# Lumina-Group/libzkp

Measured on AMD Instinct MI355X. Metric: proofs/sec (whole node) + ms/proof p50, 4096-proof mixed batch (range / equality / membership / improvement) per MI355X, higher is better.
Workload: dtype u32/u64 integer limbs (10x25.5-bit GF(2^255-19), BN254 Fq on 9x29-bit limbs in the MSM loops and 10x26-bit elsewhere, 8x32-bit Fr and scalars mod l, 2x64-bit f128)

## Files before the change

libzkp_amd/csrc/batch_impl.inc:

```
namespace {

struct PackView {
    uint32_t n;
    const uint64_t* src_off;
    const uint32_t* len_fixed;
    const uint32_t* dyn_ix;
    const uint8_t* dyn_kind;
    const int32_t* status_fixed;
    const uint32_t* dyn_len; const int32_t* dyn_status;
    uint32_t* len; int32_t* status; uint64_t* out_off;
    const uint8_t* arena; uint8_t* out;
};
__global__ void __launch_bounds__(256) k_batch_lens(PackView P) {
    const uint32_t i = blockIdx.x * 256 + threadIdx.x;
    if (i >= P.n) return;
    int32_t st = P.status_fixed[i];
    uint32_t l = P.len_fixed[i];
    if (st == 0 && l == LEN_DYN) {
        const uint32_t k = P.dyn_ix[i];
        l = P.dyn_len[k];
        if (P.dyn_kind[i] == DYN_LEN_STATUS) st = P.dyn_status[k];
        else if (l == 0) st = ZKP_HIP_PROOF_GENERATION_FAILED;
    }
    if (st != 0) l = 0;
// ... 190 lines not shown
    hipStream_t st = dev().stream;
    if (P.in_bytes) HIP_TRY(hipMemcpyAsync(P.d_in, h, P.in_bytes, hipMemcpyHostToDevice, st));
    HIP_TRY(hipStreamSynchronize(st));
    return 0;
}

PackView pack_view(const ShardPlan& P) {
    uint8_t *in = P.d_in, *ar = P.d_arena;
    PackView V{};
    V.n = P.n; V.src_off = (const uint64_t*)(in + P.i_src); V.len_fixed = (const uint32_t*)(in + P.i_lenf); V.dyn_ix = (const uint32_t*)(in + P.i_dix);
    V.dyn_kind = in + P.i_dkind; V.status_fixed = (const int32_t*)(in + P.i_stf); V.dyn_len = (const uint32_t*)(ar + P.a_dlen); V.dyn_status = (const int32_t*)(ar + P.a_dst);
    V.len = (uint32_t*)(P.d_meta + P.m_len); V.status = (int32_t*)(P.d_meta + P.m_status); V.out_off = (uint64_t*)(P.d_meta + P.m_off);
    V.arena = ar; V.out = P.d_out;
    return V;
}

int launch_shard_enqueue(ShardPlan& P) {
    BatchState* BS = nullptr; int rc;
    if ((rc = batch_state(&BS))) return rc;
    const uint32_t n = P.n;
    uint32_t lane_ix = 0;
    if ((rc = pick_lane(*BS, &lane_ix))) return rc;
    BatchLane& LN = BS->lane[lane_ix];
    hipStream_t st = LN.main;
    uint8_t *in = P.d_in, *ar = P.d_arena;
    const VariantPlan &R = P.var[ZKP_HIP_OP_RANGE], &E = P.var[ZKP_HIP_OP_EQUALITY], &T = P.var[ZKP_HIP_OP_THRESHOLD], &M = P.var[ZKP_HIP_OP_MEMBERSHIP],
                      &I = P.var[ZKP_HIP_OP_IMPROVEMENT], &C = P.var[ZKP_HIP_OP_CONSISTENCY];
    trace_origin(st);
    if (P.arena_bytes) HIP_TRY(hipMemsetAsync(ar, 0, P.arena_bytes, st));
    if (T.rows) HIP_TRY(hipMemcpyAsync(ar + T.arena, P.thr_img.data(), P.thr_img.size(), hipMemcpyHostToDevice, st));
    if (C.rows) HIP_TRY(hipMemcpyAsync(ar + C.arena, P.con_img.data(), P.con_img.size(), hipMemcpyHostToDevice, st));
    HIP_TRY(hipEventRecord(LN.go, st));
    bool used[4] = {false, false, false, false};
    auto on_stream = [&](int k, auto body) -> int {
        hipStream_t s = nullptr; used[k] = true;
        int rcs;
        if ((rcs = lane_stream(*BS, k, &s))) return rcs;
        HIP_TRY(hipStreamWaitEvent(s, LN.go, 0));
        if ((rcs = body(s))) return rcs;
        HIP_TRY(hipEventRecord(LN.done[k], s));
        return 0;
    };
    if (R.rows || T.rows || C.rows) {
        static const int edg_prio = env_int("ZKP_HIP_EDG_PRIORITY", 1);
        struct PrioScope { int& r; PrioScope(int& ref, int v) : r(ref) { r = v; } ~PrioScope() { r = 0; } };
        PrioScope prio(dev().msm_prio_now, (E.rows + M.rows) && edg_prio ? 1 : 0);
        SubBatch& jobs_sb = dev().sub[0];
        if ((rc = on_stream(0, [&](hipStream_t s) -> int {
                int rcb;
                if (R.rows && (rcb = prove_range_device_locked(R.rows, (const uint64_t*)(in + P.i_rv), (const uint64_t*)(in + P.i_rmin), (const uint64_t*)(in + P.i_rmax), 6, in + P.i_rseed,
                                                               ar + R.arena, R.stride, (uint32_t*)(ar + P.a_dlen), (int32_t*)(ar + P.a_dst), s, nullptr, (int)lane_ix))) return rcb;
                if (T.rows && (rcb = run_jobs_on(jobs_sb, P.thrJ, in + P.i_tseed, ar + T.arena, 6, s))) return rcb;
                if (C.rows) {
                    if ((rcb = run_jobs_on(jobs_sb, P.conJ, in + P.i_cseed, ar + C.arena, 6, s))) return rcb;
                    k_consistency_digest<<<(C.rows + 63) / 64, 64, 0, s>>>(ar + C.arena, C.stride, (const uint32_t*)(in + P.i_ccount), (const uint32_t*)(in + P.i_clen), C.rows);
                }
                return 0;
            }))) return rc;
    }
    if (I.rows && (rc = on_stream(3, [&](hipStream_t s) -> int {
            if (const int rcb = ensure_stark_constants()) return rcb;
            ZKP_TRACED("k_stark_prove", s, stark_launch_prove((const uint64_t*)(in + P.i_io), (const uint64_t*)(in + P.i_in), I.rows, g_stark_const, ar + I.arena, I.stride,
                                                              (uint32_t*)(ar + P.a_dlen) + R.rows, s));
            return 0;
        }))) return rc;
    if (M.rows && (rc = on_stream(2, [&](hipStream_t s) {
            return run_g16(G16_MEMBERSHIP, M.rows, (const uint64_t*)(in + P.i_mv), (const uint64_t*)(in + P.i_msets), (const uint32_t*)(in + P.i_mlen), in + P.i_mseed,
                           ar + M.arena, M.stride, s, lane_ix);
        }))) return rc;
    if (E.rows && (rc = on_stream(1, [&](hipStream_t s) {
            return run_g16(G16_EQUALITY, E.rows, (const uint64_t*)(in + P.i_ev), nullptr, nullptr, in + P.i_eseed, ar + E.arena, E.stride, s, lane_ix);
        }))) return rc;
    for (int k = 0; k < 4; k++) if (used[k]) HIP_TRY(hipStreamWaitEvent(st, LN.done[k], 0));
    const PackView V = pack_view(P);
    if (n && P.self_check) {
    } else if (n) {
        ZKP_TRACED("k_batch_lens+scan+pack", st, k_batch_lens<<<(n + 255) / 256, 256, 0, st>>>(V); k_batch_scan<<<1, 1024, 0, st>>>(V); k_batch_pack<<<n, 256, 0, st>>>(V));
    } else {
        HIP_TRY(hipMemsetAsync(P.d_meta + P.m_off, 0, 8, st));
    }
    HIP_TRY(hipGetLastError());
    HIP_TRY(hipEventRecord(P.finished, st));
    HIP_TRY(hipEventRecord(LN.idle, st)); LN.used = true;
    P.in_flight = true;
    return 0;
}
int launch_shard(ShardPlan& P) {
    if (P.generation != dev().generation) return fail(ZKP_HIP_E_ARGUMENT, "the batch was staged before zkp_hip_shutdown: stage it again");
    if (P.var[ZKP_HIP_OP_EQUALITY].rows && !g16s().key[G16_EQUALITY].loaded) return no_proving_key(g16s().key[G16_EQUALITY]);
    if (P.var[ZKP_HIP_OP_MEMBERSHIP].rows && !g16s().key[G16_MEMBERSHIP].loaded) return no_proving_key(g16s().key[G16_MEMBERSHIP]);
    const int rc = launch_shard_enqueue(P);
    if (rc) {
        const std::string keep = t_err;
        (void)hipDeviceSynchronize();
        t_err = keep;
    }
    return rc;
}
int self_check_shard(ShardPlan& P) {
    const auto t0 = std::chrono::steady_clock::now();
    const uint32_t n = P.n;
    hipStream_t st = dev().stream;
    uint8_t *in = P.d_in, *ar = P.d_arena;
    const PackView W = pack_view(P);
    SelfCheckView V{};
// ... 282 lines not shown
```

libzkp_amd/csrc/g16_impl.inc:

```

namespace {

struct G16Key {
    bool loaded = false;
    uint32_t n_inst = 0, n_wit = 0, nv = 0, n_rows = 0, m = 0, logm = 0;
    G16Circuit C{};
    std::vector<void*> allocs;
    uint32_t *table_g1 = nullptr, *table_g2 = nullptr;
    G16Radix rx = g16_radix(G16_WBITS_DEFAULT);
    int shared_tables = -1;
    uint64_t table_bytes = 0;
    struct Chunking { DevLayout lay; const uint32_t* corr = nullptr; const uint16_t* scal = nullptr; };
    std::vector<SlotList> targets_g1, targets_g2;
    std::vector<uint16_t> hscal_g1, hscal_g2;
    std::map<uint64_t, Chunking> lays_g1, lays_g2;
    uint64_t win_g1 = 0, win_g2 = 0;
    const uint32_t *init_g1 = nullptr, *init_g2 = nullptr;
    G16Vk vk{}; bool vk_ready = false;
    uint64_t vk_table_bytes = 0;
    bool verifier_only() const { return vk_ready && !loaded; }
    const uint32_t *vm_kconst = nullptr, *vm_lines = nullptr;
};
struct G16Run {
    void* buf = nullptr; size_t cap = 0; hipStream_t side = nullptr, side2 = nullptr; hipEvent_t ev[4] = {nullptr, nullptr, nullptr, nullptr};
// ... 350 lines not shown
    for (uint32_t k = 0; k < nv; k++) s2.push_back(Bt[k]);
    std::vector<uint8_t> b1, b2; int rc;
    if ((rc = gpu_scalar_mults(false, s1, b1)) || (rc = gpu_scalar_mults(true, s2, b2))) return rc;
    auto g1at = [&](size_t i) { return b1.data() + 64 * i; };
    auto g2at = [&](size_t i) { return b2.data() + 128 * i; };
    auto put = [](std::vector<uint8_t>& v, const uint8_t* p, size_t n) { v.insert(v.end(), p, p + n); };
    auto put_len = [](std::vector<uint8_t>& v, uint64_t n) { for (int i = 0; i < 8; i++) v.push_back((uint8_t)(n >> (8 * i))); };
    size_t o_abc = 3, o_a = o_abc + T.n_inst, o_b = o_a + nv, o_h = o_b + nv, o_l = o_h + (m - 1);
    vk.clear();
    put(vk, g1at(0), 64); put(vk, g2at(0), 128); put(vk, g2at(1), 128); put(vk, g2at(2), 128);
    put_len(vk, T.n_inst); put(vk, g1at(o_abc), 64ull * T.n_inst);
    pk = vk;
    put(pk, g1at(1), 64); put(pk, g1at(2), 64);
    put_len(pk, nv); put(pk, g1at(o_a), 64ull * nv);
    put_len(pk, nv); put(pk, g1at(o_b), 64ull * nv);
    put_len(pk, nv); put(pk, g2at(3), 128ull * nv);
    put_len(pk, m - 1); put(pk, g1at(o_h), 64ull * (m - 1));
    put_len(pk, T.n_wit); put(pk, g1at(o_l), 64ull * T.n_wit);
    return load_key_locked(kind, pk.data(), pk.size());
}

int launch_msm_key(bool g2, const G16Radix& rx, const G16Key::Chunking& ch, const uint32_t* table, const uint32_t* acc_init, uint32_t rows, const uint32_t* digits, uint32_t* partial, hipStream_t st) {
    const DevLayout& D = ch.lay;
    const MsmView m = g16_msm_view(rx, D, ch.scal, table, acc_init, rows, digits, partial);
    Device::KProf& K = dev().prof[g2 ? 2 : 1];
    hipEvent_t e1 = nullptr;
    int rc = prof_begin(K, st, &e1);
    if (rc) return rc;
    ZKP_TRACED(g2 ? "k_msm_gather<G2Msm>" : "k_msm_gather<G1Msm>", st, g16_launch_msm(g2, m, st));
    prof_end(K, st, e1, D.adds_per_row * rows);
    return 0;
}


int run_g16(int kind, uint32_t rows, const uint64_t* d_value, const uint64_t* d_set_vals, const uint32_t* d_set_len, const uint8_t* d_seeds,
            uint8_t* d_out, uint64_t stride, hipStream_t st, uint32_t lane = 0) {
    G16Key& K = g16s().key[kind];
    if (!K.loaded) return no_proving_key(K);
    const uint32_t nsc = g16_nscalars(K.nv, K.m);
    const G16Key::Chunking *c1 = nullptr, *c1c = nullptr, *c2 = nullptr;
    int rc;
    if ((rc = get_chunking(K, false, G16_PART_AB, rows, &c1)) || (rc = get_chunking(K, true, G16_PART_ALL, rows, &c2))) return rc;
    if ((rc = get_chunking(K, false, G16_PART_C, rows, &c1c))) return rc;
    size_t off = 0;
    auto sz = [&](size_t bytes) { size_t o = off; off += align_up(bytes); return o; };
    const size_t W = (size_t)32 * rows;
    const size_t o_z = sz(W * K.nv), o_sd = sz((size_t)K.rx.digw * 4 * rows * nsc), o_rs = sz(W * 2), o_p1 = sz((size_t)c1->lay.nchunks * G1_JAC_W * 4 * rows),
                 o_p1c = sz((size_t)c1c->lay.nchunks * G1_JAC_W * 4 * rows), o_p2 = sz((size_t)c2->lay.nchunks * G2_JAC_W * 4 * rows),
                 o_s1 = sz((size_t)3 * G1_JAC_W * 4 * rows), o_s2 = sz((size_t)G2_JAC_W * 4 * rows), o_t1 = sz((size_t)G16_CPARTS * G1_JAC_W * 4 * rows),
                 o_qe = sz((size_t)2 * 9 * K.m * 4 * rows);
    G16Run& RW = g16s().run[kind][lane & 1u];
    if (off > RW.cap) {
        if (RW.buf) { HIP_TRY(hipDeviceSynchronize()); HIP_TRY(hipFree(RW.buf)); RW.buf = nullptr; RW.cap = 0; }
        HIP_TRY(hipMalloc(&RW.buf, off)); RW.cap = off;
    }
    uint8_t* base = (uint8_t*)RW.buf;
    G16View V{}; V.rx = K.rx; V.rows = rows; V.kind = (uint32_t)kind; V.n_inst = K.n_inst; V.n_wit = K.n_wit; V.nv = K.nv; V.m = K.m;
    V.value = d_value; V.set_vals = d_set_vals; V.set_len = d_set_len; V.seeds = reinterpret_cast<const uint32_t*>(d_seeds); V.mimc_c = g16s().mimc_dev;
    V.z = (uint32_t*)(base + o_z); V.sdig = (uint32_t*)(base + o_sd); V.rs = (uint32_t*)(base + o_rs); V.out = d_out; V.stride = stride;
    V.qap_evals = (uint32_t*)(base + o_qe);
    uint32_t *p1 = (uint32_t*)(base + o_p1), *p1c = (uint32_t*)(base + o_p1c), *p2 = (uint32_t*)(base + o_p2), *s1 = (uint32_t*)(base + o_s1), *s2 = (uint32_t*)(base + o_s2), *t1 = (uint32_t*)(base + o_t1);
    if (!RW.last) {
        for (auto& e : RW.ev) HIP_TRY(hipEventCreateWithFlags(&e, hipEventDisableTiming));
        HIP_TRY(hipEventCreateWithFlags(&RW.last, hipEventDisableTiming));
    }
    G16Run& R0 = g16s().run[kind][0];
    if (!R0.side) {
        static const int side_level = env_int("ZKP_HIP_G16_SIDE_PRIORITY", 2), side2_level = env_int("ZKP_HIP_G16_SIDE2_PRIORITY", 0);
        HIP_TRY(hipStreamCreateWithPriority(&R0.side, hipStreamNonBlocking, stream_priority(side_level)));
        HIP_TRY(hipStreamCreateWithPriority(&R0.side2, hipStreamNonBlocking, stream_priority(side2_level)));
    }
    hipStream_t const side = R0.side, side2 = R0.side2;
    hipEvent_t ev_wit = RW.ev[0], ev_ab = RW.ev[1], ev_c = RW.ev[2], ev_cp = RW.ev[3];
    ReduceView R2{}; R2.rows = rows; R2.ntargets = 1; R2.partial = p2; R2.target_chunk_begin = c2->lay.target_chunk_begin; R2.corr = c2->corr;
    if (RW.used) HIP_TRY(hipStreamWaitEvent(st, RW.last, 0));
    ZKP_TRACED("k_g16_witness", st, g16_launch_witness(V, st));
    ZKP_TRACED("k_g16_zdigits", st, g16_launch_zdigits(V, st));
    HIP_TRY(hipEventRecord(ev_wit, st));
    HIP_TRY(hipStreamWaitEvent(side, ev_wit, 0));
    { TraceMark tm_("k_g16_qap", side); HIP_TRY(g16_launch_qap(V, K.C, side)); }
    if ((rc = launch_msm_key(false, K.rx, *c1c, K.table_g1, K.init_g1, rows, V.sdig, p1c, side))) return rc;
    ReduceView Rc{}; Rc.rows = rows; Rc.ntargets = 1; Rc.partial = p1c; Rc.target_chunk_begin = c1c->lay.target_chunk_begin; Rc.corr = c1c->corr;
    ZKP_TRACED("k_sum_t<G1Msm>", side, g16_launch_sum(false, Rc, s1 + (size_t)2 * G1_JAC_W * rows, side));
    HIP_TRY(hipEventRecord(ev_c, side));
    if ((rc = launch_msm_key(false, K.rx, *c1, K.table_g1, K.init_g1, rows, V.sdig, p1, st))) return rc;
    ReduceView Rab{}; Rab.rows = rows; Rab.ntargets = 2; Rab.partial = p1; Rab.target_chunk_begin = c1->lay.target_chunk_begin; Rab.corr = c1->corr;
    if (c1->lay.ntargets == 3) Rab.target_chunk_end = c1->lay.target_chunk_begin + 2;
    HIP_TRY(hipEventRecord(ev_ab, st));
    HIP_TRY(hipStreamWaitEvent(side2, ev_ab, 0));
    ZKP_TRACED("k_sum_t<G1Msm>", side2, g16_launch_sum(false, Rab, s1, side2));
    ZKP_TRACED("k_g16_cparts", side2, g16_launch_cparts(V, s1, t1, side2));
    HIP_TRY(hipEventRecord(ev_cp, side2));
    if ((rc = launch_msm_key(true, K.rx, *c2, K.table_g2, K.init_g2, rows, V.sdig, p2, st))) return rc;
    ZKP_TRACED("k_sum_t<G2Msm>", st, g16_launch_sum(true, R2, s2, st));
    HIP_TRY(hipStreamWaitEvent(st, ev_c, 0));
    HIP_TRY(hipStreamWaitEvent(st, ev_cp, 0));
    ZKP_TRACED("k_g16_final", st, g16_launch_final(V, s1, s2, t1, st));
    HIP_TRY(hipGetLastError());
    HIP_TRY(hipEventRecord(RW.last, st)); RW.used = true;
    return 0;
}

int prove_g16_host(int kind, uint64_t n, const uint64_t* values, const uint64_t* sets_flat, const uint32_t* set_counts, const std::vector<uint8_t>& valid,
                   const uint8_t* seeds, uint8_t* out, uint64_t stride, uint32_t* out_len, int32_t* status) {
    if (g16s().key[kind].verifier_only()) return no_proving_key(g16s().key[kind]);
    std::vector<uint64_t> v, sv; std::vector<uint32_t> sl, idx; std::vector<uint8_t> sd;
    size_t pos = 0; int any = 0;
    memset(out, 0, stride * n);
    for (uint64_t i = 0; i < n; i++) {
        const uint32_t cnt = set_counts ? set_counts[i] : 0;
        if (valid[i]) {
            idx.push_back((uint32_t)i); v.push_back(values[i]);
            sd.insert(sd.end(), seeds + 32 * i, seeds + 32 * i + 32);
            if (kind == G16_MEMBERSHIP) { sl.push_back(cnt); for (uint32_t k = 0; k < G16_MAX_SET; k++) sv.push_back(k < cnt ? sets_flat[pos + k] : 0); }
            const uint32_t plen = kind == G16_EQUALITY ? EQUALITY_ENVELOPE_BYTES : (uint32_t)membership_envelope_bytes(cnt);
            if (plen > stride) return fail(ZKP_HIP_E_ARGUMENT, "stride too small for the proof envelope");
            out_len[i] = plen; status[i] = ZKP_HIP_OK;
        } else { out_len[i] = 0; status[i] = ZKP_HIP_INVALID_INPUT; any = 1; }
        pos += cnt;
    }
    const uint32_t rows = (uint32_t)idx.size();
    if (rows == 0) return any;
    hipStream_t st = dev().stream;
    uint64_t *d_v = nullptr, *d_sv = nullptr; uint32_t* d_sl = nullptr; uint8_t *d_sd = nullptr, *d_out = nullptr;
    DevScope mem;
    HIP_TRY(mem.alloc(&d_v, 8ull * rows)); HIP_TRY(mem.alloc(&d_sd, 32ull * rows)); HIP_TRY(mem.alloc(&d_out, stride * rows));
    HIP_TRY(hipMemcpyAsync(d_v, v.data(), 8ull * rows, hipMemcpyHostToDevice, st));
    HIP_TRY(hipMemcpyAsync(d_sd, sd.data(), 32ull * rows, hipMemcpyHostToDevice, st));
    HIP_TRY(hipMemsetAsync(d_out, 0, stride * rows, st));
    if (kind == G16_MEMBERSHIP) {
        HIP_TRY(mem.alloc(&d_sv, 8ull * sv.size())); HIP_TRY(mem.alloc(&d_sl, 4ull * rows));
        HIP_TRY(hipMemcpyAsync(d_sv, sv.data(), 8ull * sv.size(), hipMemcpyHostToDevice, st));
        HIP_TRY(hipMemcpyAsync(d_sl, sl.data(), 4ull * rows, hipMemcpyHostToDevice, st));
// ... 284 lines not shown
```

libzkp_amd/csrc/g16_kernels.hip:

```cpp
#include "g16_launch.h"
#include "msm_kernel.h"

struct G1Msm {
    static constexpr uint32_t ACC_W = G1_JAC_W, DIG_PER_WORD = 2;
    static __device__ __forceinline__ int32_t digit(uint32_t word, uint32_t w) { return (int32_t)(int16_t)(word >> (16 * (w & 1u))); }
    using Acc = g1_jac;
    static __device__ __forceinline__ Acc identity() { return jac_infinity<fq>(); }
    static constexpr uint32_t GATHER_WAVES = 3; static constexpr int GATHER_PREFETCH = 2;
    static constexpr uint32_t GATHER_W = 16, GATHER_STRIDE = 16, GATHER_PRIO = 0;
    using GAcc = g1_xyzz9;
    static __device__ __forceinline__ GAcc to_gather(const g1_jac& a) { return xyzz9_from_jac(a); }
    static __device__ __forceinline__ g1_jac from_gather(const GAcc& a) { return jac_from_xyzz9(a); }
    static __device__ __forceinline__ GAcc accumulate_entry(const GAcc& acc, int32_t d, const uint32_t* e) {
        g1_aff9 q{fq9_unpack8(e), fq9_unpack8(e + 8)};
        q.y = fq9_select(d < 0, fq9_neg_k<4>(q.y), q.y);
        return g1_mmadd9(acc, q);
    }
    static __device__ __forceinline__ void store(uint32_t* p, uint32_t idx, uint32_t row, uint32_t rows, const Acc& a) { st_g1_jac(p, idx, row, rows, a); }
    static __device__ __forceinline__ Acc load(const uint32_t* p, uint32_t idx, uint32_t row, uint32_t rows) { return ld_g1_jac(p, idx, row, rows); }
    static __device__ __forceinline__ Acc add(const Acc& a, const Acc& b) { return jac_add(a, b); }
};
struct G2Msm {
    static constexpr uint32_t ACC_W = G2_JAC_W, DIG_PER_WORD = 2;
    static __device__ __forceinline__ int32_t digit(uint32_t word, uint32_t w) { return (int32_t)(int16_t)(word >> (16 * (w & 1u))); }
    using Acc = g2_jac;
    static __device__ __forceinline__ Acc identity() { return jac_infinity<fq2>(); }
    static constexpr uint32_t GATHER_WAVES = 2; static constexpr int GATHER_PREFETCH = -1;
    static constexpr uint32_t GATHER_W = 32, GATHER_STRIDE = 32, GATHER_PRIO = 0;
    using GAcc = g2_xyzz9;
    static __device__ __forceinline__ GAcc to_gather(const g2_jac& a) { return g2_xyzz9_from_jac(a); }
    static __device__ __forceinline__ g2_jac from_gather(const GAcc& a) { return jac_from_g2_xyzz9(a); }
    static __device__ __forceinline__ GAcc accumulate_entry(const GAcc& acc, int32_t d, const uint32_t* e) {
        const g2_aff9 q{fq2_9{fq9_unpack8(e), fq9_unpack8(e + 8)}, fq2_9{fq9_unpack8(e + 16), fq9_unpack8(e + 24)}};
        return g2_mmadd9(acc, q, d < 0);
    }
    static __device__ __forceinline__ void store(uint32_t* p, uint32_t idx, uint32_t row, uint32_t rows, const Acc& a) { st_g2_jac(p, idx, row, rows, a); }
    static __device__ __forceinline__ Acc load(const uint32_t* p, uint32_t idx, uint32_t row, uint32_t rows) { return ld_g2_jac(p, idx, row, rows); }
    static __device__ __forceinline__ Acc add(const Acc& a, const Acc& b) { return jac_add(a, b); }
};


__global__ void __launch_bounds__(TW) k_g16_witness(G16View V) {
    ZKP_RAISE_PRIO();
    const uint32_t row = blockIdx.x * TW + threadIdx.x;
    if (row < V.rows) step_g16_witness(V, row);
}
__global__ void __launch_bounds__(TB) k_g16_zdigits(G16View V) {
    ZKP_RAISE_PRIO();
    const uint32_t row = blockIdx.x * TB + threadIdx.x;
    if (row < V.rows) step_g16_zdigits(V, blockIdx.y, row);
}
struct DevSync { __device__ __forceinline__ void operator()() const { __syncthreads(); } };
static constexpr int QAP_TB_MAX = 256;
__global__ void __launch_bounds__(QAP_TB_MAX) k_g16_qap(G16View V, G16Circuit C) {
    extern __shared__ uint32_t g16_lds[];
    G16Lds L; L.base = g16_lds; L.m = C.m;
    g16_qap_proof(V, C, L, V.qap_evals + (size_t)blockIdx.x * 2 * 9 * C.m, blockIdx.x, threadIdx.x, blockDim.x, DevSync());
}
__global__ void __launch_bounds__(TW) k_g16_cparts(G16View V, const uint32_t* sum_g1, uint32_t* tmp_g1) {
    ZKP_RAISE_PRIO();
    const uint32_t row = blockIdx.x * TW + threadIdx.x;
    if (row < V.rows) step_g16_cparts(V, sum_g1, tmp_g1, blockIdx.y, row);
}
__global__ void __launch_bounds__(TW) k_g16_final(G16View V, const uint32_t* sum_g1, const uint32_t* sum_g2, const uint32_t* tmp_g1) {
    ZKP_RAISE_PRIO();
    const uint32_t row = blockIdx.x * TW + threadIdx.x;
    if (row < V.rows) step_g16_final(V, sum_g1, sum_g2, tmp_g1, blockIdx.y, row);
}
__global__ void __launch_bounds__(TW) k_mimc_commit(const uint64_t* values, uint32_t n, const uint32_t* mimc_c, uint8_t* out) {
    const uint32_t i = blockIdx.x * TW + threadIdx.x;
    if (i >= n) return;
    G16View V{}; V.mimc_c = mimc_c; V.z = nullptr;
    const fr h = g16_mimc_chain(V, 0, fp_from_u64<FrParams>(values[i]), 0);
    uint32_t w[8]; fp_to_raw(w, h);
    g16_put_bytes(out + 32ull * i, w, 8);
}
constexpr uint32_t G16_TABLE_SEG = 512;
template <class F, uint32_t AFF_W>
// ... 33 lines not shown
            const F zi = k ? f_mul(inv, zp[k - 1]) : inv;
            if (k) inv = f_mul(inv, pts[k].Z);
            const F zi2 = f_sq(zi);
            Aff<F> a; a.x = f_mul(pts[k].X, zi2); a.y = f_mul(pts[k].Y, f_mul(zi2, zi));
            const uint32_t* ax = reinterpret_cast<const uint32_t*>(&a.x); const uint32_t* ay = reinterpret_cast<const uint32_t*>(&a.y);
            uint32_t* o = dst + (size_t)(e0 + k) * OW;
            if (fmt9) {
                const fq* c = reinterpret_cast<const fq*>(&a);
                for (uint32_t t2 = 0; t2 < NC; t2++) fq9_pack8(o + 8 * t2, fq9_from_fq(c[t2]));
                continue;
            }
            for (uint32_t j = 0; j < FW; j++) { o[j] = ax[j]; o[FW + j] = ay[j]; }
        }
    }
}



__global__ void __launch_bounds__(TW) k_g16_serialize(bool g2, const uint32_t* jac, uint32_t rows, uint8_t* out) {
    const uint32_t row = blockIdx.x * TW + threadIdx.x;
    if (row >= rows) return;
    if (!g2) { uint32_t w[16]; g1_serialize(w, ld_g1_jac(jac, 0, row, rows)); g16_put_bytes(out + 64ull * row, w, 16); }
    else { uint32_t w[32]; g2_serialize(w, ld_g2_jac(jac, 0, row, rows)); g16_put_bytes(out + 128ull * row, w, 32); }
}

template __global__ void k_msm_gather<G1Msm>(MsmView, uint32_t, uint32_t);
template __global__ void k_msm_gather<G2Msm>(MsmView, uint32_t, uint32_t);
static constexpr uint32_t G16_SUM_ROWS = 8, G16_SUM_TB = 256;
template __global__ void k_sum_t<G1Msm, G16_SUM_ROWS, G16_SUM_TB>(ReduceView, uint32_t*);
template __global__ void k_sum_t<G2Msm, G16_SUM_ROWS, G16_SUM_TB>(ReduceView, uint32_t*);
template __global__ void k_g16_build_table<fq, 20>(const uint32_t*, uint32_t, uint32_t*, uint32_t, G16Radix);
template __global__ void k_g16_build_table<fq2, 40>(const uint32_t*, uint32_t, uint32_t*, uint32_t, G16Radix);

void g16_launch_witness(const G16View& V, hipStream_t st) { k_g16_witness<<<(V.rows + TW - 1) / TW, TW, 0, st>>>(V); }
void g16_launch_zdigits(const G16View& V, hipStream_t st) { k_g16_zdigits<<<dim3((V.rows + TB - 1) / TB, V.nv), TB, 0, st>>>(V); }
hipError_t g16_launch_qap(const G16View& V, const G16Circuit& C, hipStream_t st) {
    const size_t lds = (size_t)9 * C.m * 4;
    const uint32_t tb = C.m / 4;
    if (tb < 64 || tb > (uint32_t)QAP_TB_MAX || (tb & 63u)) return hipErrorInvalidValue;
    k_g16_qap<<<V.rows, tb, lds, st>>>(V, C);
    return hipSuccess;
}
void g16_launch_cparts(const G16View& V, const uint32_t* sum_g1, uint32_t* tmp_g1, hipStream_t st) {
    k_g16_cparts<<<dim3((V.rows + TW - 1) / TW, G16_CPARTS), TW, 0, st>>>(V, sum_g1, tmp_g1);
}
void g16_launch_final(const G16View& V, const uint32_t* sum_g1, const uint32_t* sum_g2, const uint32_t* tmp_g1, hipStream_t st) {
    k_g16_final<<<dim3((V.rows + TW - 1) / TW, 3), TW, 0, st>>>(V, sum_g1, sum_g2, tmp_g1);
}
void g16_launch_mimc(const uint64_t* values, uint32_t n, const uint32_t* mimc_c, uint8_t* out, hipStream_t st) { k_mimc_commit<<<(n + TW - 1) / TW, TW, 0, st>>>(values, n, mimc_c, out); }
void g16_launch_build_table(bool g2, const uint32_t* bases, uint32_t nslots, uint32_t* table, hipStream_t st, bool msm_form, const G16Radix& rx) {
    const uint32_t seg_len = rx.nent < G16_TABLE_SEG ? rx.nent : G16_TABLE_SEG;
    const uint32_t threads = nslots * (rx.slot_ent / seg_len);
    if (!g2) k_g16_build_table<fq, 20><<<(threads + TW - 1) / TW, TW, 0, st>>>(bases, nslots, table, msm_form ? 1u : 0u, rx);
    else k_g16_build_table<fq2, 40><<<(threads + TW - 1) / TW, TW, 0, st>>>(bases, nslots, table, msm_form ? 1u : 0u, rx);
}
uint32_t g16_table_entry_words(bool g2, bool msm_form) { return msm_form ? (g2 ? G2Msm::GATHER_W : G1Msm::GATHER_W) : (g2 ? 40u : 20u); }
uint32_t g16_msm_rows_per_block(bool) { return 256u; }
uint32_t g16_msm_blocks_per_cu(bool g2) { return g2 ? G2Msm::GATHER_WAVES : G1Msm::GATHER_WAVES; }
void g16_launch_msm(bool g2, const MsmView& m, hipStream_t st) {
    const uint32_t ngroups = (m.rows + 255u) / 256u, nblocks = m.nchunks * ngroups, grid = ((nblocks + 7) / 8) * 8;
    if constexpr (gather_lds_bytes<G2Msm>() > 0 || gather_lds_bytes<G1Msm>() > 0) {
        if (gather_lds_bytes<G1Msm>()) (void)hipFuncSetAttribute(reinterpret_cast<const void*>(k_msm_gather<G1Msm>), hipFuncAttributeMaxDynamicSharedMemorySize, (int)gather_lds_bytes<G1Msm>());
        if (gather_lds_bytes<G2Msm>()) (void)hipFuncSetAttribute(reinterpret_cast<const void*>(k_msm_gather<G2Msm>), hipFuncAttributeMaxDynamicSharedMemorySize, (int)gather_lds_bytes<G2Msm>());
    }
    if (!g2) k_msm_gather<G1Msm><<<grid, 256, gather_lds_bytes<G1Msm>(), st>>>(m, ngroups, nblocks);
    else k_msm_gather<G2Msm><<<grid, 256, gather_lds_bytes<G2Msm>(), st>>>(m, ngroups, nblocks);
}
// ... 7 lines not shown
```

libzkp_amd/csrc/g16_steps.h:

```cpp
#pragma once
#include "bn254_g.h"
#include "bn254_fr9.h"
#include "keccak.h"
#include "sc25519.h"

namespace zkp {

struct G16Radix { uint32_t wbits, nwin, nent, digw, nwin_u64, uneven, slot_ent; };
constexpr uint32_t G16_UNEVEN_TOP_ENT = 25088;
ZKP_HD inline G16Radix g16_radix(uint32_t wbits, bool uneven = false) {
    G16Radix r; r.wbits = wbits; r.nwin = (254 + wbits) / wbits; r.nent = 1u << (wbits - 1); r.nwin_u64 = (64 + wbits) / wbits; r.uneven = 0;
    r.slot_ent = r.nwin * r.nent;
    if (uneven && wbits == 14) { r.uneven = 1; r.nwin = 18; r.slot_ent = 18u * r.nent + G16_UNEVEN_TOP_ENT; }
    r.digw = (r.nwin + 1) / 2;
    return r;
}
ZKP_HD inline uint32_t g16_win_bit(const G16Radix& rx, uint32_t w) { return rx.uneven && w == 17 ? 239u : rx.wbits * w; }
ZKP_HD inline uint32_t g16_win_off(const G16Radix& rx, uint32_t w) { return (w + (rx.uneven && w == 17 ? 1u : 0u)) * rx.nent; }
ZKP_HD inline uint32_t g16_win_ent(const G16Radix& rx, uint32_t w) { return !rx.uneven || w < 16 ? rx.nent : w == 16 ? 2u * rx.nent : G16_UNEVEN_TOP_ENT; }
constexpr uint32_t G16_WBITS_DEFAULT = 14, G16_WBITS_KNEE = 13, G16_WBITS_MIN = 8, G16_WBITS_MAX = 15, G16_DIGW_MAX = 16;
static_assert(G16_WBITS_DEFAULT >= G16_WBITS_MIN && G16_WBITS_DEFAULT <= G16_WBITS_MAX, "key-table radix out of range");
ZKP_HD inline void g16_recode_uneven(uint32_t* packed, const sc& raw) {
    uint32_t carry = 0;
    ZKP_UNROLL for (int j = 0; j < 18; j++) {
// ... 47 lines not shown

struct G16View {
    uint32_t rows, kind;
    G16Radix rx;
    uint32_t n_inst, n_wit, nv, m;
    const uint64_t* value;
    const uint64_t* set_vals;
    const uint32_t* set_len;
    const uint32_t* seeds;
    const uint32_t* mimc_c;
    uint32_t* z;
    uint32_t* sdig;
    uint32_t* rs;
    uint32_t* qap_evals;
    uint8_t* out; uint64_t stride;
};
ZKP_HD inline uint32_t g16_sc_h(const G16View& V) { return V.nv; }
ZKP_HD inline uint32_t g16_sc_r(const G16View& V) { return V.nv + V.m - 1; }
ZKP_HD inline uint32_t g16_sc_s(const G16View& V) { return V.nv + V.m; }
ZKP_HD inline uint32_t g16_sc_nrs(const G16View& V) { return V.nv + V.m + 1; }
ZKP_HD inline uint32_t g16_sc_one(const G16View& V) { return V.nv + V.m + 2; }
ZKP_HD inline uint32_t g16_nscalars(uint32_t nv, uint32_t m) { return nv + m + 3; }

ZKP_HD inline fr g16_mimc_chain(const G16View& V, uint32_t row, fr x, uint32_t wit0) {
    for (uint32_t i = 0; i < MIMC_ROUNDS; i++) {
        const fr t = fp_add(x, ld_fr_c(V.mimc_c, i));
        const fr t2 = fp_sq(t), t4 = fp_sq(t2);
        x = fp_mul(t4, t);
        if (V.z) { st_fr(V.z, wit0 + 3 * i, row, V.rows, t2); st_fr(V.z, wit0 + 3 * i + 1, row, V.rows, t4); st_fr(V.z, wit0 + 3 * i + 2, row, V.rows, x); }
    }
    return x;
}

ZKP_HD inline void step_g16_witness(const G16View& V, uint32_t row) {
    const uint32_t rows = V.rows;
    const uint64_t val = V.value[row];
    const fr one = fp_one<FrParams>(), zero = fp_zero<FrParams>();
    const fr v = fp_from_u64<FrParams>(val);
    uint8_t* o = V.out + (uint64_t)row * V.stride;
    st_fr(V.z, 0, row, rows, one);
    fr h;
    uint32_t proof_len = 256;
    if (V.kind == G16_EQUALITY) {
        st_fr(V.z, 2, row, rows, v); st_fr(V.z, 3, row, rows, v);
        h = g16_mimc_chain(V, row, v, 4);
        st_fr(V.z, 1, row, rows, h);
        o[0] = 2; o[1] = 2;
    } else {
        const uint32_t len = V.set_len[row];
        const uint64_t* sv = V.set_vals + (size_t)row * G16_MAX_SET;
        const uint32_t w0 = V.n_inst;
        st_fr(V.z, w0, row, rows, v);
        h = g16_mimc_chain(V, row, v, w0 + 1);
        st_fr(V.z, 1, row, rows, h);
        uint32_t pos = 0xffffffffu;
        for (uint32_t i = 0; i < len; i++) if (pos == 0xffffffffu && sv[i] == val) pos = i;
        const uint32_t sel0 = w0 + 1 + 3 * MIMC_ROUNDS;
        for (uint32_t i = 0; i < G16_MAX_SET; i++) {
            const bool real = i < len;
            const fr si = fp_from_u64<FrParams>(real ? sv[i] : 0);
            st_fr(V.z, 2 + i, row, rows, si);
            st_fr(V.z, 2 + G16_MAX_SET + i, row, rows, real ? one : zero);
            const bool sel = i == pos;
            st_fr(V.z, sel0 + i, row, rows, sel ? one : zero);
            st_fr(V.z, sel0 + G16_MAX_SET + i, row, rows, (sel && !real) ? one : zero);
            st_fr(V.z, sel0 + 2 * G16_MAX_SET + i, row, rows, sel ? fp_sub(v, si) : zero);
        }
        o[0] = 2; o[1] = 4;
        proof_len = 4 + 8 * len + 256;
        uint8_t* pl = o + 10;
        pl[0] = (uint8_t)len; pl[1] = (uint8_t)(len >> 8); pl[2] = (uint8_t)(len >> 16); pl[3] = (uint8_t)(len >> 24);
        for (uint32_t i = 0; i < len; i++) for (int k = 0; k < 8; k++) pl[4 + 8 * i + k] = (uint8_t)(sv[i] >> (8 * k));
    }
    for (int k = 0; k < 4; k++) { o[2 + k] = (uint8_t)(proof_len >> (8 * k)); o[6 + k] = (uint8_t)(32u >> (8 * k)); }
    uint32_t hraw[8]; fp_to_raw(hraw, h);
    g16_put_bytes(o + 10 + proof_len, hraw, 8);
    uint32_t seed[8]; ZKP_UNROLL for (int k = 0; k < 8; k++) seed[k] = V.seeds[(size_t)row * 8 + k];
    uint32_t w[16];
    tape_draw64(w, seed, G16_TAPE_IDX, 0); const fr r = fp_from_wide<FrParams>(w);
    tape_draw64(w, seed, G16_TAPE_IDX, 1); const fr s = fp_from_wide<FrParams>(w);
    st_fr_digits(V.sdig, g16_sc_r(V), row, rows, r, V.rx);
    st_fr_digits(V.sdig, g16_sc_s(V), row, rows, s, V.rx);
    st_fr_digits(V.sdig, g16_sc_nrs(V), row, rows, fp_neg(fp_mul(r, s)), V.rx);
    uint32_t* q = V.sdig + (size_t)g16_sc_one(V) * V.rx.digw * rows + row;
    q[0] = 1u; for (uint32_t k = 1; k < V.rx.digw; k++) q[(size_t)k * rows] = 0u;
    fr rr, sr; fp_to_raw(rr.v, r); fp_to_raw(sr.v, s);
    st_fr(V.rs, 0, row, rows, rr); st_fr(V.rs, 1, row, rows, sr);
}
ZKP_HD inline void step_g16_zdigits(const G16View& V, uint32_t k, uint32_t row) {
    st_fr_digits(V.sdig, k, row, V.rows, ld_fr(V.z, k, row, V.rows), V.rx);
}

struct G16Circuit {
    uint32_t n_rows, m, logm;
    const uint32_t *a_ptr, *a_col, *a_coef, *b_ptr, *b_col, *b_coef, *c_ptr, *c_col, *c_coef;
    const uint32_t *tw, *tw_inv;
    const uint32_t *coset, *coset_inv;
    const uint32_t* zinv;
};
ZKP_HD inline fr g16_row_dot(const uint32_t* ptr, const uint32_t* col, const uint32_t* coef, uint32_t r, const uint32_t* z, uint32_t row, uint32_t rows) {
    fr acc = fp_zero<FrParams>();
    for (uint32_t e = ptr[r]; e < ptr[r + 1]; e++) acc = fp_add(acc, fp_mul(ld_fr_c(coef, e), ld_fr(z, col[e], row, rows)));
    return acc;
}
ZKP_HD inline uint32_t g16_bitrev(uint32_t x, uint32_t bits) {
    uint32_t r = 0; for (uint32_t i = 0; i < bits; i++) { r = (r << 1) | (x & 1u); x >>= 1; } return r;
}

struct G16Lds {
    uint32_t* base; uint32_t m;
    ZKP_HD static uint32_t sw(uint32_t e) { return e ^ ((0u - ((e >> 5) & 1u)) & 10u) ^ ((0u - ((e >> 6) & 1u)) & 21u); }
    ZKP_HD fr9 ld(uint32_t e) const { fr9 r; const uint32_t p = sw(e); ZKP_UNROLL for (int k = 0; k < 9; k++) r.v[k] = base[(size_t)k * m + p]; return r; }
    ZKP_HD void st(uint32_t e, const fr9& v) const { const uint32_t p = sw(e); ZKP_UNROLL for (int k = 0; k < 9; k++) base[(size_t)k * m + p] = v.v[k]; }
};
ZKP_HD inline fr9 ld_fr9_c(const uint32_t* p, uint32_t idx) { fr9 r; ZKP_UNROLL for (int k = 0; k < 9; k++) r.v[k] = p[(size_t)idx * 9 + k]; return r; }
ZKP_HD inline fr g16_row_dot_fast(const uint32_t* ptr, const uint32_t* col, const uint32_t* coef, uint32_t r, const uint32_t* z, uint32_t row, uint32_t rows) {
    const fr one = fp_one<FrParams>();
    fr acc = fp_zero<FrParams>();
    for (uint32_t e = ptr[r]; e < ptr[r + 1]; e++) {
        const fr cf = ld_fr_c(coef, e);
// ... 139 lines not shown
```

Measured before the change: 347,100.

## Enqueue Groth16 witness head before range jobs and split witness kernel into parallel parts

Splits run_g16 into a head (witness and zdigits) and a body (QAP, MSMs). For small equality/membership batches the heads are enqueued before the range/threshold/consistency work, so the serial witness stage starts early and overlaps with other streams. The witness kernel also gains a grid y-dimension that computes the MiMC chain, the randomness draw and each set element in separate threads instead of one long serial thread. This adds recomputation of the membership position check per element and changes the order in which streams receive work.

```diff
diff --git a/libzkp_amd/csrc/batch_impl.inc b/libzkp_amd/csrc/batch_impl.inc
--- a/libzkp_amd/csrc/batch_impl.inc
+++ b/libzkp_amd/csrc/batch_impl.inc
@@ -246,15 +246,41 @@
     if (C.rows) HIP_TRY(hipMemcpyAsync(ar + C.arena, P.con_img.data(), P.con_img.size(), hipMemcpyHostToDevice, st));
     HIP_TRY(hipEventRecord(LN.go, st));
     bool used[4] = {false, false, false, false};
-    auto on_stream = [&](int k, auto body) -> int {
-        hipStream_t s = nullptr; used[k] = true;
-        int rcs;
-        if ((rcs = lane_stream(*BS, k, &s))) return rcs;
-        HIP_TRY(hipStreamWaitEvent(s, LN.go, 0));
-        if ((rcs = body(s))) return rcs;
-        HIP_TRY(hipEventRecord(LN.done[k], s));
+    auto open_stream = [&](int k, hipStream_t* s) -> int {
+        used[k] = true;
+        if (const int rcs = lane_stream(*BS, k, s)) return rcs;
+        HIP_TRY(hipStreamWaitEvent(*s, LN.go, 0));
         return 0;
     };
+    auto close_stream = [&](int k, hipStream_t s) -> int { HIP_TRY(hipEventRecord(LN.done[k], s)); return 0; };
+    auto on_stream = [&](int k, auto body) -> int {
+        hipStream_t s = nullptr;
+        int rcs;
+        if ((rcs = open_stream(k, &s)) || (rcs = body(s))) return rcs;
+        return close_stream(k, s);
+    };
+    static const int g16_head_first_rows = env_int("ZKP_HIP_G16_HEAD_FIRST", 2048);
+    const bool g16_head_first = g16_head_first_rows > 0 && (uint64_t)E.rows + M.rows <= (uint64_t)g16_head_first_rows;
+    struct G16Phase { hipStream_t s = nullptr; G16Head H; bool open = false; } g16_mem, g16_eq;
+    auto g16_head = [&](G16Phase& G, int kind) -> int {
+        const int k = kind == G16_MEMBERSHIP ? 2 : 1;
+        if (const int rcs = open_stream(k, &G.s)) return rcs;
+        G.open = true;
+        if (kind == G16_MEMBERSHIP)
+            return run_g16_head(G16_MEMBERSHIP, M.rows, (const uint64_t*)(in + P.i_mv), (const uint64_t*)(in + P.i_msets), (const uint32_t*)(in + P.i_mlen), in + P.i_mseed,
+                                ar + M.arena, M.stride, G.s, lane_ix, G.H);
+        return run_g16_head(G16_EQUALITY, E.rows, (const uint64_t*)(in + P.i_ev), nullptr, nullptr, in + P.i_eseed, ar + E.arena, E.stride, G.s, lane_ix, G.H);
+    };
+    auto g16_body = [&](G16Phase& G, int kind) -> int {
+        int rcs;
+        if (!G.open && (rcs = g16_head(G, kind))) return rcs;
+        if ((rcs = run_g16_body(G.H, G.s))) return rcs;
+        return close_stream(kind == G16_MEMBERSHIP ? 2 : 1, G.s);
+    };
+    if (g16_head_first) {
+        if (M.rows && (rc = g16_head(g16_mem, G16_MEMBERSHIP))) return rc;
+        if (E.rows && (rc = g16_head(g16_eq, G16_EQUALITY))) return rc;
+    }
     if (R.rows || T.rows || C.rows) {
         static const int edg_prio = env_int("ZKP_HIP_EDG_PRIORITY", 1);
         struct PrioScope { int& r; PrioScope(int& ref, int v) : r(ref) { r = v; } ~PrioScope() { r = 0; } };
@@ -278,13 +304,8 @@
                                                               (uint32_t*)(ar + P.a_dlen) + R.rows, s));
             return 0;
         }))) return rc;
-    if (M.rows && (rc = on_stream(2, [&](hipStream_t s) {
-            return run_g16(G16_MEMBERSHIP, M.rows, (const uint64_t*)(in + P.i_mv), (const uint64_t*)(in + P.i_msets), (const uint32_t*)(in + P.i_mlen), in + P.i_mseed,
-                           ar + M.arena, M.stride, s, lane_ix);
-        }))) return rc;
-    if (E.rows && (rc = on_stream(1, [&](hipStream_t s) {
-            return run_g16(G16_EQUALITY, E.rows, (const uint64_t*)(in + P.i_ev), nullptr, nullptr, in + P.i_eseed, ar + E.arena, E.stride, s, lane_ix);
-        }))) return rc;
+    if (M.rows && (rc = g16_body(g16_mem, G16_MEMBERSHIP))) return rc;
+    if (E.rows && (rc = g16_body(g16_eq, G16_EQUALITY))) return rc;
     for (int k = 0; k < 4; k++) if (used[k]) HIP_TRY(hipStreamWaitEvent(st, LN.done[k], 0));
     const PackView V = pack_view(P);
     if (n && P.self_check) {
diff --git a/libzkp_amd/csrc/g16_impl.inc b/libzkp_amd/csrc/g16_impl.inc
--- a/libzkp_amd/csrc/g16_impl.inc
+++ b/libzkp_amd/csrc/g16_impl.inc
@@ -406,21 +406,26 @@
     return 0;
 }
 
-
-int run_g16(int kind, uint32_t rows, const uint64_t* d_value, const uint64_t* d_set_vals, const uint32_t* d_set_len, const uint8_t* d_seeds,
-            uint8_t* d_out, uint64_t stride, hipStream_t st, uint32_t lane = 0) {
+struct G16Head {
+    int kind = 0; uint32_t rows = 0, lane = 0;
+    G16View V{};
+    const G16Key::Chunking *c1 = nullptr, *c1c = nullptr, *c2 = nullptr;
+    uint32_t *p1 = nullptr, *p1c = nullptr, *p2 = nullptr, *s1 = nullptr, *s2 = nullptr, *t1 = nullptr;
+};
+int run_g16_head(int kind, uint32_t rows, const uint64_t* d_value, const uint64_t* d_set_vals, const uint32_t* d_set_len, const uint8_t* d_seeds,
+                 uint8_t* d_out, uint64_t stride, hipStream_t st, uint32_t lane, G16Head& H) {
     G16Key& K = g16s().key[kind];
     if (!K.loaded) return no_proving_key(K);
     const uint32_t nsc = g16_nscalars(K.nv, K.m);
-    const G16Key::Chunking *c1 = nullptr, *c1c = nullptr, *c2 = nullptr;
+    H.kind = kind; H.rows = rows; H.lane = lane;
     int rc;
-    if ((rc = get_chunking(K, false, G16_PART_AB, rows, &c1)) || (rc = get_chunking(K, true, G16_PART_ALL, rows, &c2))) return rc;
-    if ((rc = get_chunking(K, false, G16_PART_C, rows, &c1c))) return rc;
+    if ((rc = get_chunking(K, false, G16_PART_AB, rows, &H.c1)) || (rc = get_chunking(K, true, G16_PART_ALL, rows, &H.c2))) return rc;
+    if ((rc = get_chunking(K, false, G16_PART_C, rows, &H.c1c))) return rc;
     size_t off = 0;
     auto sz = [&](size_t bytes) { size_t o = off; off += align_up(bytes); return o; };
     const size_t W = (size_t)32 * rows;
-    const size_t o_z = sz(W * K.nv), o_sd = sz((size_t)K.rx.digw * 4 * rows * nsc), o_rs = sz(W * 2), o_p1 = sz((size_t)c1->lay.nchunks * G1_JAC_W * 4 * rows),
-                 o_p1c = sz((size_t)c1c->lay.nchunks * G1_JAC_W * 4 * rows), o_p2 = sz((size_t)c2->lay.nchunks * G2_JAC_W * 4 * rows),
+    const size_t o_z = sz(W * K.nv), o_sd = sz((size_t)K.rx.digw * 4 * rows * nsc), o_rs = sz(W * 2), o_p1 = sz((size_t)H.c1->lay.nchunks * G1_JAC_W * 4 * rows),
+                 o_p1c = sz((size_t)H.c1c->lay.nchunks * G1_JAC_W * 4 * rows), o_p2 = sz((size_t)H.c2->lay.nchunks * G2_JAC_W * 4 * rows),
                  o_s1 = sz((size_t)3 * G1_JAC_W * 4 * rows), o_s2 = sz((size_t)G2_JAC_W * 4 * rows), o_t1 = sz((size_t)G16_CPARTS * G1_JAC_W * 4 * rows),
                  o_qe = sz((size_t)2 * 9 * K.m * 4 * rows);
     G16Run& RW = g16s().run[kind][lane & 1u];
@@ -429,11 +434,13 @@
         HIP_TRY(hipMalloc(&RW.buf, off)); RW.cap = off;
     }
     uint8_t* base = (uint8_t*)RW.buf;
-    G16View V{}; V.rx = K.rx; V.rows = rows; V.kind = (uint32_t)kind; V.n_inst = K.n_inst; V.n_wit = K.n_wit; V.nv = K.nv; V.m = K.m;
+    G16View& V = H.V;
+    V = G16View{}; V.rx = K.rx; V.rows = rows; V.kind = (uint32_t)kind; V.n_inst = K.n_inst; V.n_wit = K.n_wit; V.nv = K.nv; V.m = K.m;
     V.value = d_value; V.set_vals = d_set_vals; V.set_len = d_set_len; V.seeds = reinterpret_cast<const uint32_t*>(d_seeds); V.mimc_c = g16s().mimc_dev;
     V.z = (uint32_t*)(base + o_z); V.sdig = (uint32_t*)(base + o_sd); V.rs = (uint32_t*)(base + o_rs); V.out = d_out; V.stride = stride;
     V.qap_evals = (uint32_t*)(base + o_qe);
-    uint32_t *p1 = (uint32_t*)(base + o_p1), *p1c = (uint32_t*)(base + o_p1c), *p2 = (uint32_t*)(base + o_p2), *s1 = (uint32_t*)(base + o_s1), *s2 = (uint32_t*)(base + o_s2), *t1 = (uint32_t*)(base + o_t1);
+    H.p1 = (uint32_t*)(base + o_p1); H.p1c = (uint32_t*)(base + o_p1c); H.p2 = (uint32_t*)(base + o_p2); H.s1 = (uint32_t*)(base + o_s1); H.s2 = (uint32_t*)(base + o_s2);
+    H.t1 = (uint32_t*)(base + o_t1);
     if (!RW.last) {
         for (auto& e : RW.ev) HIP_TRY(hipEventCreateWithFlags(&e, hipEventDisableTiming));
         HIP_TRY(hipEventCreateWithFlags(&RW.last, hipEventDisableTiming));
@@ -444,13 +451,24 @@
         HIP_TRY(hipStreamCreateWithPriority(&R0.side, hipStreamNonBlocking, stream_priority(side_level)));
         HIP_TRY(hipStreamCreateWithPriority(&R0.side2, hipStreamNonBlocking, stream_priority(side2_level)));
     }
-    hipStream_t const side = R0.side, side2 = R0.side2;
-    hipEvent_t ev_wit = RW.ev[0], ev_ab = RW.ev[1], ev_c = RW.ev[2], ev_cp = RW.ev[3];
-    ReduceView R2{}; R2.rows = rows; R2.ntargets = 1; R2.partial = p2; R2.target_chunk_begin = c2->lay.target_chunk_begin; R2.corr = c2->corr;
+    hipEvent_t ev_wit = RW.ev[0];
     if (RW.used) HIP_TRY(hipStreamWaitEvent(st, RW.last, 0));
     ZKP_TRACED("k_g16_witness", st, g16_launch_witness(V, st));
     ZKP_TRACED("k_g16_zdigits", st, g16_launch_zdigits(V, st));
     HIP_TRY(hipEventRecord(ev_wit, st));
+    return 0;
+}
+int run_g16_body(const G16Head& H, hipStream_t st) {
+    G16Key& K = g16s().key[H.kind];
+    const G16View& V = H.V;
+    const uint32_t rows = H.rows;
+    const G16Key::Chunking *c1 = H.c1, *c1c = H.c1c, *c2 = H.c2;
+    uint32_t *p1 = H.p1, *p1c = H.p1c, *p2 = H.p2, *s1 = H.s1, *s2 = H.s2, *t1 = H.t1;
+    G16Run &RW = g16s().run[H.kind][H.lane & 1u], &R0 = g16s().run[H.kind][0];
+    hipStream_t const side = R0.side, side2 = R0.side2;
+    hipEvent_t ev_wit = RW.ev[0], ev_ab = RW.ev[1], ev_c = RW.ev[2], ev_cp = RW.ev[3];
+    ReduceView R2{}; R2.rows = rows; R2.ntargets = 1; R2.partial = p2; R2.target_chunk_begin = c2->lay.target_chunk_begin; R2.corr = c2->corr;
+    int rc;
     HIP_TRY(hipStreamWaitEvent(side, ev_wit, 0));
     { TraceMark tm_("k_g16_qap", side); HIP_TRY(g16_launch_qap(V, K.C, side)); }
     if ((rc = launch_msm_key(false, K.rx, *c1c, K.table_g1, K.init_g1, rows, V.sdig, p1c, side))) return rc;
@@ -473,6 +491,12 @@
     HIP_TRY(hipGetLastError());
     HIP_TRY(hipEventRecord(RW.last, st)); RW.used = true;
     return 0;
+}
+int run_g16(int kind, uint32_t rows, const uint64_t* d_value, const uint64_t* d_set_vals, const uint32_t* d_set_len, const uint8_t* d_seeds,
+            uint8_t* d_out, uint64_t stride, hipStream_t st, uint32_t lane = 0) {
+    G16Head H;
+    if (const int rc = run_g16_head(kind, rows, d_value, d_set_vals, d_set_len, d_seeds, d_out, stride, st, lane, H)) return rc;
+    return run_g16_body(H, st);
 }
 
 int prove_g16_host(int kind, uint64_t n, const uint64_t* values, const uint64_t* sets_flat, const uint32_t* set_counts, const std::vector<uint8_t>& valid,
diff --git a/libzkp_amd/csrc/g16_kernels.hip b/libzkp_amd/csrc/g16_kernels.hip
--- a/libzkp_amd/csrc/g16_kernels.hip
+++ b/libzkp_amd/csrc/g16_kernels.hip
@@ -43,7 +43,10 @@
 __global__ void __launch_bounds__(TW) k_g16_witness(G16View V) {
     ZKP_RAISE_PRIO();
     const uint32_t row = blockIdx.x * TW + threadIdx.x;
-    if (row < V.rows) step_g16_witness(V, row);
+    if (row >= V.rows) return;
+    if (blockIdx.y == 0) step_g16_witness_chain(V, row);
+    else if (blockIdx.y == 1) step_g16_witness_rand(V, row);
+    else step_g16_witness_set(V, row, blockIdx.y - 2);
 }
 __global__ void __launch_bounds__(TB) k_g16_zdigits(G16View V) {
     ZKP_RAISE_PRIO();
@@ -143,7 +146,10 @@
 template __global__ void k_g16_build_table<fq, 20>(const uint32_t*, uint32_t, uint32_t*, uint32_t, G16Radix);
 template __global__ void k_g16_build_table<fq2, 40>(const uint32_t*, uint32_t, uint32_t*, uint32_t, G16Radix);
 
-void g16_launch_witness(const G16View& V, hipStream_t st) { k_g16_witness<<<(V.rows + TW - 1) / TW, TW, 0, st>>>(V); }
+void g16_launch_witness(const G16View& V, hipStream_t st) {
+    const uint32_t parts = V.kind == G16_MEMBERSHIP ? 2 + G16_MAX_SET : 2;
+    k_g16_witness<<<dim3((V.rows + TW - 1) / TW, parts), TW, 0, st>>>(V);
+}
 void g16_launch_zdigits(const G16View& V, hipStream_t st) { k_g16_zdigits<<<dim3((V.rows + TB - 1) / TB, V.nv), TB, 0, st>>>(V); }
 hipError_t g16_launch_qap(const G16View& V, const G16Circuit& C, hipStream_t st) {
     const size_t lds = (size_t)9 * C.m * 4;
diff --git a/libzkp_amd/csrc/g16_steps.h b/libzkp_amd/csrc/g16_steps.h
--- a/libzkp_amd/csrc/g16_steps.h
+++ b/libzkp_amd/csrc/g16_steps.h
@@ -103,13 +103,11 @@
     return x;
 }
 
-ZKP_HD inline void step_g16_witness(const G16View& V, uint32_t row) {
+ZKP_HD inline void step_g16_witness_chain(const G16View& V, uint32_t row) {
     const uint32_t rows = V.rows;
-    const uint64_t val = V.value[row];
-    const fr one = fp_one<FrParams>(), zero = fp_zero<FrParams>();
-    const fr v = fp_from_u64<FrParams>(val);
+    const fr v = fp_from_u64<FrParams>(V.value[row]);
     uint8_t* o = V.out + (uint64_t)row * V.stride;
-    st_fr(V.z, 0, row, rows, one);
+    st_fr(V.z, 0, row, rows, fp_one<FrParams>());
     fr h;
     uint32_t proof_len = 256;
     if (V.kind == G16_EQUALITY) {
@@ -119,33 +117,21 @@
         o[0] = 2; o[1] = 2;
     } else {
         const uint32_t len = V.set_len[row];
-        const uint64_t* sv = V.set_vals + (size_t)row * G16_MAX_SET;
         const uint32_t w0 = V.n_inst;
         st_fr(V.z, w0, row, rows, v);
         h = g16_mimc_chain(V, row, v, w0 + 1);
         st_fr(V.z, 1, row, rows, h);
-        uint32_t pos = 0xffffffffu;
-        for (uint32_t i = 0; i < len; i++) if (pos == 0xffffffffu && sv[i] == val) pos = i;
-        const uint32_t sel0 = w0 + 1 + 3 * MIMC_ROUNDS;
-        for (uint32_t i = 0; i < G16_MAX_SET; i++) {
-            const bool real = i < len;
-            const fr si = fp_from_u64<FrParams>(real ? sv[i] : 0);
-            st_fr(V.z, 2 + i, row, rows, si);
-            st_fr(V.z, 2 + G16_MAX_SET + i, row, rows, real ? one : zero);
-            const bool sel = i == pos;
-            st_fr(V.z, sel0 + i, row, rows, sel ? one : zero);
-            st_fr(V.z, sel0 + G16_MAX_SET + i, row, rows, (sel && !real) ? one : zero);
-            st_fr(V.z, sel0 + 2 * G16_MAX_SET + i, row, rows, sel ? fp_sub(v, si) : zero);
-        }
         o[0] = 2; o[1] = 4;
         proof_len = 4 + 8 * len + 256;
         uint8_t* pl = o + 10;
         pl[0] = (uint8_t)len; pl[1] = (uint8_t)(len >> 8); pl[2] = (uint8_t)(len >> 16); pl[3] = (uint8_t)(len >> 24);
-        for (uint32_t i = 0; i < len; i++) for (int k = 0; k < 8; k++) pl[4 + 8 * i + k] = (uint8_t)(sv[i] >> (8 * k));
     }
     for (int k = 0; k < 4; k++) { o[2 + k] = (uint8_t)(proof_len >> (8 * k)); o[6 + k] = (uint8_t)(32u >> (8 * k)); }
     uint32_t hraw[8]; fp_to_raw(hraw, h);
     g16_put_bytes(o + 10 + proof_len, hraw, 8);
+}
+ZKP_HD inline void step_g16_witness_rand(const G16View& V, uint32_t row) {
+    const uint32_t rows = V.rows;
     uint32_t seed[8]; ZKP_UNROLL for (int k = 0; k < 8; k++) seed[k] = V.seeds[(size_t)row * 8 + k];
     uint32_t w[16];
     tape_draw64(w, seed, G16_TAPE_IDX, 0); const fr r = fp_from_wide<FrParams>(w);
@@ -157,6 +143,32 @@
     q[0] = 1u; for (uint32_t k = 1; k < V.rx.digw; k++) q[(size_t)k * rows] = 0u;
     fr rr, sr; fp_to_raw(rr.v, r); fp_to_raw(sr.v, s);
     st_fr(V.rs, 0, row, rows, rr); st_fr(V.rs, 1, row, rows, sr);
+}
+ZKP_HD inline void step_g16_witness_set(const G16View& V, uint32_t row, uint32_t i) {
+    const uint32_t rows = V.rows, len = V.set_len[row];
+    const uint64_t val = V.value[row];
+    const uint64_t* sv = V.set_vals + (size_t)row * G16_MAX_SET;
+    const fr one = fp_one<FrParams>(), zero = fp_zero<FrParams>();
+    const bool real = i < len;
+    const uint64_t svi = sv[i];
+    bool sel = real && svi == val;
+    for (uint32_t j = 0; j < i; j++) if (sv[j] == val) sel = false;
+    const fr si = fp_from_u64<FrParams>(real ? svi : 0);
+    const uint32_t sel0 = V.n_inst + 1 + 3 * MIMC_ROUNDS;
+    st_fr(V.z, 2 + i, row, rows, si);
+    st_fr(V.z, 2 + G16_MAX_SET + i, row, rows, real ? one : zero);
+    st_fr(V.z, sel0 + i, row, rows, sel ? one : zero);
+    st_fr(V.z, sel0 + G16_MAX_SET + i, row, rows, (sel && !real) ? one : zero);
+    st_fr(V.z, sel0 + 2 * G16_MAX_SET + i, row, rows, sel ? fp_sub(fp_from_u64<FrParams>(val), si) : zero);
+    if (real) {
+        uint8_t* pl = V.out + (uint64_t)row * V.stride + 10;
+        for (int k = 0; k < 8; k++) pl[4 + 8 * i + k] = (uint8_t)(svi >> (8 * k));
+    }
+}
+ZKP_HD inline void step_g16_witness(const G16View& V, uint32_t row) {
+    step_g16_witness_chain(V, row);
+    step_g16_witness_rand(V, row);
+    if (V.kind == G16_MEMBERSHIP) for (uint32_t i = 0; i < G16_MAX_SET; i++) step_g16_witness_set(V, row, i);
 }
 ZKP_HD inline void step_g16_zdigits(const G16View& V, uint32_t k, uint32_t row) {
     st_fr_digits(V.sdig, k, row, V.rows, ld_fr(V.z, k, row, V.rows), V.rx);
```

Result: no change. 351,000, median of 2 (+1.1%).
